# sampotter/butterfly

Hardware: AMD Instinct MI355X
Metric: butterfly matvecs/sec (2D Helmholtz HODBF apply) (higher is better)
Workload: dtype c128

## Files before the change

### butterfly_amd/csrc/bfhip_device.hip

```cpp

#include <hip/hip_runtime.h>
#include <type_traits>
#include <vector>
#include <stdint.h>
#include <stdio.h>
#include <stdlib.h>

#include "bfhip_internal.h"
#include "bfhip_stage_c128.h"
#include "../../include/bfhip_abi.h"
#include "../../include/bfhip_synth.h"

#define BF_WAVES_PER_WG 4
#define BF_WAVE_LDS_BYTES (BF_XCAP * 16)

static int hipFail(hipError_t e, char const *what) {
  if (e == hipSuccess) return 0;
  int code = (e == hipErrorOutOfMemory) ? BFABI_ERROR_MEMORY_ERROR : BFABI_ERROR_RUNTIME_ERROR;
  return bfhipFail(code, "%s: %s", what, hipGetErrorString(e));
}

struct __attribute__((aligned(8))) bfC64 { float re, im; };
struct bfC64Acc { double re, im; };
__device__ __forceinline__ bfC64Acc &operator+=(bfC64Acc &a, bfC64Acc b) { a.re += b.re; a.im += b.im; return a; }
// ... 519 lines not shown
            bool dual = pi + pstep < wn;
            BfDevPiece pc2 = pc;
            if (dual) {
              pc2 = bfPieceWinGet(win, pi + pstep);
              dual = (pc2.flags & (BF_PIECE_ROWMAJOR | BF_PIECE_IDENTITY)) == BF_PIECE_ROWMAJOR;
            }
            U a[ITERS], a2[ITERS];
            S xv[ITERS][NC], xv2[ITERS][NC];
#pragma unroll
            for (int i = 0; i < ITERS; ++i) {
              uint32_t const srow = rlRm + (uint32_t)i * RL_RM, sc = srow < n ? srow : n - 1;
              a[i] = bfLoadStreamV(src + (uint64_t)sc * rowUnits);
#pragma unroll
              for (int k = 0; k < NC; ++k) {
                S const xr = xin[(uint64_t)sc * nrhs * NC + k];
                xv[i][k] = srow < n ? xr : (S)0;
              }
            }
            if (dual) {
              S const *xin2 = ((pc2.flags & BF_PIECE_IN_X) ? (S const *)p.x : (S const *)p.temp) + ((uint64_t)pc2.inOff * nrhs + q) * NC;
              uint32_t const n2 = pc2.ncols;
              U const *src2 = arena + pc2.dataOff / EPL + cgc;
              uint32_t const rowUnits2 = pc2.ld / EPL;
#pragma unroll
              for (int i = 0; i < ITERS; ++i) {
                uint32_t const srow = rlRm + (uint32_t)i * RL_RM, sc = srow < n2 ? srow : n2 - 1;
                a2[i] = bfLoadStreamV(src2 + (uint64_t)sc * rowUnits2);
#pragma unroll
                for (int k = 0; k < NC; ++k) {
                  S const xr = xin2[(uint64_t)sc * nrhs * NC + k];
                  xv2[i][k] = srow < n2 ? xr : (S)0;
                }
              }
            }
#pragma unroll
            for (int i = 0; i < ITERS; ++i)
#pragma unroll
              for (int e = 0; e < EPL; ++e) bfMacN<NC>(racc[e], &a[i].v[e * NC], xv[i]);
            if (dual) {
#pragma unroll
              for (int i = 0; i < ITERS; ++i)
#pragma unroll
                for (int e = 0; e < EPL; ++e) bfMacN<NC>(racc[e], &a2[i].v[e * NC], xv2[i]);
              pi += pstep;
            }
            continue;
          }
        }
        uint32_t const stride = pc.ld / EPL;
        uint32_t const n = pc.ncols;
        uint32_t const units = (n + EPL - 1) / EPL;
        U const *src = arena + pc.dataOff / EPL;
        for (uint32_t rb = 0; rb < units; rb += R) {
          uint32_t const ru = rb + r < units ? rb + r : units - 1;
          U a[NQ];
#pragma unroll
          for (int cq = 0; cq < NQ; ++cq) if ((uint32_t)cq < nq) a[cq] = (R >= 16 || BF_T_WIDE_NT) ? bfLoadStreamV(src + jcol[cq] * stride + ru) : src[jcol[cq] * stride + ru];
          S xv[UNIT];
#pragma unroll
          for (int e = 0; e < EPL; ++e) {
            uint32_t const row = (rb + r) * EPL + e;
            uint32_t const rowc = row < n ? row : n - 1;
#pragma unroll
            for (int k = 0; k < NC; ++k) {
              S const v = xin[(uint64_t)rowc * nrhs * NC + k];
              xv[e * NC + k] = row < n ? v : (S)0;
            }
          }
#pragma unroll
          for (int cq = 0; cq < NQ; ++cq) {
            if ((uint32_t)cq >= nq) continue;
#pragma unroll
            for (int e = 0; e < EPL; ++e) bfMacN<NC>(acc[cq], &a[cq].v[e * NC], &xv[e * NC]);
          }
        }
      }
    }
#pragma unroll
    for (int m = 1; m < R; m <<= 1)
#pragma unroll
      for (int cq = 0; cq < NQ; ++cq)
#pragma unroll
        for (int k = 0; k < NC; ++k) acc[cq][k] += __shfl_xor(acc[cq][k], m, R);
    if constexpr (EPL > 1) {
      if (anyRowMajor) {
#pragma unroll
        for (int e = 0; e < EPL; ++e)
#pragma unroll
          for (int k = 0; k < NC; ++k)
#pragma unroll
            for (int m = CG_RM; m < 64; m <<= 1) racc[e][k] += __shfl_xor(racc[e][k], m, 64);
#pragma unroll
        for (int cq = 0; cq < NQ; ++cq) {
          uint32_t const col = c4 + C * cq < mr ? c4 + C * cq : 0;
#pragma unroll
          for (int e = 0; e < EPL; ++e)
#pragma unroll
            for (int k = 0; k < NC; ++k) {
              A const t = __shfl(racc[e][k], (int)(col / EPL), 64);
              if ((int)(col % EPL) == e) acc[cq][k] += t;
            }
        }
      }
    }
    if (COOP && coop) {
      if (r == 0) {
#pragma unroll
        for (int cq = 0; cq < NQ; ++cq)
#pragma unroll
          for (int k = 0; k < NC; ++k) coopBuf[wave][c4 + C * cq][k] = acc[cq][k];
      }
      __syncthreads();
      if (wave == 0 && r == 0) {
#pragma unroll
        for (int cq = 0; cq < NQ; ++cq)
#pragma unroll
          for (int k = 0; k < NC; ++k) {
            A t = coopBuf[0][c4 + C * cq][k];
#pragma unroll
            for (int w = 1; w < BF_WAVES_PER_WG; ++w) t += coopBuf[w][c4 + C * cq][k];
            acc[cq][k] = t;
          }
      }
      __syncthreads();
      if (wave != 0) continue;
    }
    if (r == 0) {
#pragma unroll
      for (int cq = 0; cq < NQ; ++cq)
        if (c4 + C * cq < mr)
#pragma unroll
          for (int k = 0; k < NC; ++k) out[(((uint64_t)it.outOff + c4 + C * cq) * nrhs + q) * NC + k] = (S)acc[cq][k];
    }
  }
}

template <int DT, int R, int NQ, bool COOP, bool ONE>
__global__ __launch_bounds__(BF_WAVES_PER_WG * 64) void bfStageKernelT(StageParams p) {
  using A = typename Traits<DT>::A;
  constexpr int NC = Traits<DT>::CPLX ? 2 : 1;
  __shared__ A coopBuf[COOP ? BF_WAVES_PER_WG : 1][COOP ? NQ * (64 / R) : 1][NC];
  bfStageBodyT<DT, R, NQ, COOP, ONE>(p, blockIdx.x, coopBuf);
}

template <int DT, bool ONE>
__global__ __launch_bounds__(BF_WAVES_PER_WG * 64) void bfStageKernelTBoth(StageParams pn, StageParams pw, uint32_t gridNarrow) {
  using A = typename Traits<DT>::A;
  constexpr int NC = Traits<DT>::CPLX ? 2 : 1;
  __shared__ A coopBuf[BF_WAVES_PER_WG][64][NC];
  if (blockIdx.x < gridNarrow) bfStageBodyT<DT, 16, 4, true, ONE>(pn, blockIdx.x, coopBuf);
  else bfStageBodyT<DT, BF_T_WIDE_R, BF_T_WIDE_R, true, ONE>(pw, blockIdx.x - gridNarrow, coopBuf);
}

struct ReduceBatch {
  uint32_t count, nrhs;
  void const *temp;
  struct Entry {
    uint32_t const *rowInterval, *ivBegin;
    int64_t const *srcBias;
    uint64_t numRows;
    void *dest;
    uint32_t blockBegin, pad;
  } e[BF_REDUCE_BATCH];
};

template <typename T, int NC, bool LONG = false>
__global__ __launch_bounds__(256) void bfReduceKernel(ReduceBatch const B) {
  using TA = typename std::conditional<NC == 2 && sizeof(T) == 4, double, T>::type;
  uint32_t k = 0;
  while (k + 1 < B.count && B.e[k + 1].blockBegin <= blockIdx.x) ++k;
  ReduceBatch::Entry const &E = B.e[k];
  uint32_t const nrhs = B.nrhs;
  uint64_t idx = (uint64_t)(blockIdx.x - E.blockBegin) * 256 + threadIdx.x;
  uint64_t total = E.numRows * nrhs;
  if (idx >= total) return;
  uint64_t row = idx / nrhs;
  uint32_t q = (uint32_t)(idx - row * nrhs);
  uint32_t iv = E.rowInterval[row];
  if (iv == 0xffffffffu) return;
  uint32_t b = E.ivBegin[iv], e = E.ivBegin[iv + 1];
  T const *temp = (T const *)B.temp;
  T *dest = (T *)E.dest;
  TA acc[NC];
#pragma unroll
  for (int c = 0; c < NC; ++c) acc[c] = 0;
  uint32_t s = b;
  if (LONG) {
    for (; s + 32 <= e; s += 32) {
      T v[32][NC];
#pragma unroll
      for (int k = 0; k < 32; ++k) {
        T const *src = temp + ((uint64_t)(E.srcBias[s + k] + (int64_t)row) * nrhs + q) * NC;
#pragma unroll
        for (int c = 0; c < NC; ++c) v[k][c] = src[c];
      }
#pragma unroll
      for (int k = 0; k < 32; ++k)
#pragma unroll
        for (int c = 0; c < NC; ++c) acc[c] += v[k][c];
    }
  }
#pragma unroll 8
  for (; s < e; ++s) {
    T const *src = temp + ((uint64_t)(E.srcBias[s] + (int64_t)row) * nrhs + q) * NC;
#pragma unroll
    for (int c = 0; c < NC; ++c) acc[c] += src[c];
  }
#pragma unroll
  for (int c = 0; c < NC; ++c) dest[idx * NC + c] = (T)acc[c];
}

template <typename S>
__global__ __launch_bounds__(256) void bfScalePermuteKernel(S *dst, S const *src, S const *scale, int power, uint64_t const *perm, uint64_t n) {
  uint64_t const i = (uint64_t)blockIdx.x * 256 + threadIdx.x;
  if (i >= n) return;
  S v = src[i];
  if (scale) { S const g = scale[i]; v *= power == 2 ? g * g : g; }
  uint64_t const j = perm ? perm[i] : i;
  if (j < n) dst[j] = v;
}

template <int DT>
__global__ __launch_bounds__(256) void bfSynthKernel(void *arenaV, BfSynthPiece const *pieces, uint64_t seed) {
  using S = typename Traits<DT>::S;
  constexpr bool CPLX = Traits<DT>::CPLX;
  BfSynthPiece const pc = pieces[blockIdx.x];
  uint64_t total = pc.rowMajor ? (uint64_t)pc.mr * pc.ldr : (uint64_t)pc.mrPad * pc.ncols;
  S *dst = (S *)arenaV + pc.dataOff * (CPLX ? 2 : 1);
  for (uint64_t e = threadIdx.x; e < total; e += 256) {
    uint32_t col, r;
    if (pc.rowMajor) { r = (uint32_t)(e / pc.ldr); col = (uint32_t)(e - (uint64_t)r * pc.ldr); }
    else { col = (uint32_t)(e / pc.mrPad); r = (uint32_t)(e - (uint64_t)col * pc.mrPad); }
    S re = 0, im = 0;
    if (r < pc.mr && col < pc.ncols) {
      uint64_t idx = pc.vbase + (uint64_t)(pc.row0 + r) * pc.strideR + (uint64_t)(pc.col0 + col) * pc.strideC;
      re = (S)(bfhip_synth_value(seed, idx, 0) * pc.scale);
      if (CPLX) im = (S)(bfhip_synth_value(seed, idx, 1) * pc.scale);
    }
    if (CPLX) { dst[2 * e] = re; dst[2 * e + 1] = im; }
    else dst[e] = re;
  }
}


#define BF_REAL_CASES(DT, NAME) \
  case BFHIP_KERNEL_REAL_##NAME: hipLaunchKernelGGL(bfStageKernelReal<DT>, dim3(grid), dim3(BF_WAVES_PER_WG * 64), 0, s, p); break; \
  case BFHIP_KERNEL_SMALL_##NAME: hipLaunchKernelGGL(bfStageKernelSmall<DT>, dim3(grid), dim3(BF_WAVES_PER_WG * 64), 0, s, p); break; \
  case BFHIP_KERNEL_REALBOTH_##NAME: hipLaunchKernelGGL(bfStageKernelRealBoth<DT>, dim3(grid + grid2), dim3(BF_WAVES_PER_WG * 64), 0, s, p, p2, grid); break;
#define BF_T_CASES(DT, NAME) \
  case BFHIP_KERNEL_T_##NAME##_NARROW_N: hipLaunchKernelGGL((bfStageKernelT<DT, 16, 4, false, false>), dim3(grid), dim3(BF_WAVES_PER_WG * 64), 0, s, p); break; \
  case BFHIP_KERNEL_T_##NAME##_NARROW_ONE: hipLaunchKernelGGL((bfStageKernelT<DT, 16, 4, false, true>), dim3(grid), dim3(BF_WAVES_PER_WG * 64), 0, s, p); break; \
  case BFHIP_KERNEL_T_##NAME##_NARROW_COOP_N: hipLaunchKernelGGL((bfStageKernelT<DT, 16, 4, true, false>), dim3(grid), dim3(BF_WAVES_PER_WG * 64), 0, s, p); break; \
  case BFHIP_KERNEL_T_##NAME##_NARROW_COOP_ONE: hipLaunchKernelGGL((bfStageKernelT<DT, 16, 4, true, true>), dim3(grid), dim3(BF_WAVES_PER_WG * 64), 0, s, p); break; \
  case BFHIP_KERNEL_T_##NAME##_WIDE_N: hipLaunchKernelGGL((bfStageKernelT<DT, BF_T_WIDE_R, BF_T_WIDE_R, false, false>), dim3(grid), dim3(BF_WAVES_PER_WG * 64), 0, s, p); break; \
  case BFHIP_KERNEL_T_##NAME##_WIDE_ONE: hipLaunchKernelGGL((bfStageKernelT<DT, BF_T_WIDE_R, BF_T_WIDE_R, false, true>), dim3(grid), dim3(BF_WAVES_PER_WG * 64), 0, s, p); break; \
  case BFHIP_KERNEL_T_##NAME##_WIDE_COOP_N: hipLaunchKernelGGL((bfStageKernelT<DT, BF_T_WIDE_R, BF_T_WIDE_R, true, false>), dim3(grid), dim3(BF_WAVES_PER_WG * 64), 0, s, p); break; \
  case BFHIP_KERNEL_T_##NAME##_WIDE_COOP_ONE: hipLaunchKernelGGL((bfStageKernelT<DT, BF_T_WIDE_R, BF_T_WIDE_R, true, true>), dim3(grid), dim3(BF_WAVES_PER_WG * 64), 0, s, p); break;
#define BF_TBOTH_CASES(DT, NAME) \
  case BFHIP_KERNEL_TBOTH_##NAME##_N: hipLaunchKernelGGL((bfStageKernelTBoth<DT, false>), dim3(grid + grid2), dim3(BF_WAVES_PER_WG * 64), 0, s, p, p2, grid); break; \
  case BFHIP_KERNEL_TBOTH_##NAME##_ONE: hipLaunchKernelGGL((bfStageKernelTBoth<DT, true>), dim3(grid + grid2), dim3(BF_WAVES_PER_WG * 64), 0, s, p, p2, grid); break;
static int bfLaunchWaveStage(BfKernelLaunch const &L, BfLaunchArgs const *a, StageParams p, hipStream_t s) {
  bool const small = L.kernel >= BFHIP_KERNEL_SMALL_F64 && L.kernel <= BFHIP_KERNEL_SMALL_C64;
  uint32_t const perWg = small ? 4 * BF_WAVES_PER_WG : BF_WAVES_PER_WG;
  p.items = (BfDevItem const *)a->items + L.first[0];
  p.numItems = (uint32_t)L.count[0];
  p.coopItems = (uint32_t)L.coop[0];
  uint32_t const grid = (uint32_t)(L.coop[0] + (L.count[0] - L.coop[0] + perWg - 1) / perWg);
  StageParams p2 = p;
  uint32_t grid2 = 0;
  if (L.numRanges == 2) {
    bool const tboth = L.kernel >= BFHIP_KERNEL_TBOTH_F64_N && L.kernel <= BFHIP_KERNEL_TBOTH_C64_ONE;
    uint32_t const perWg2 = tboth ? BF_WAVES_PER_WG : 4 * BF_WAVES_PER_WG;
    p2.items = (BfDevItem const *)a->items + L.first[1];
    p2.numItems = (uint32_t)L.count[1];
    p2.coopItems = (uint32_t)L.coop[1];
    grid2 = (uint32_t)(L.coop[1] + (L.count[1] - L.coop[1] + perWg2 - 1) / perWg2);
  }
  switch (L.kernel) {
    BF_REAL_CASES(BFHIP_F64, F64) BF_REAL_CASES(BFHIP_F32, F32) BF_REAL_CASES(BFHIP_C64, C64)
    BF_T_CASES(BFHIP_C128, C128) BF_T_CASES(BFHIP_F64, F64) BF_T_CASES(BFHIP_F32, F32) BF_T_CASES(BFHIP_C64, C64)
    BF_TBOTH_CASES(BFHIP_F64, F64) BF_TBOTH_CASES(BFHIP_F32, F32) BF_TBOTH_CASES(BFHIP_C64, C64)
    default: return bfhipFail(BFABI_ERROR_RUNTIME_ERROR, "internal: kernel id %u is not a wavefront-per-item stage kernel", L.kernel);
  }
  return 0;
}
#undef BF_REAL_CASES
#undef BF_T_CASES
#undef BF_TBOTH_CASES

extern "C" {

int bfdevSetDevice(int device) {
  if (device < 0) return 0;
  return hipFail(hipSetDevice(device), "hipSetDevice");
}
int bfdevGetDevice(int *device) { return hipFail(hipGetDevice(device), "hipGetDevice"); }
int bfdevMalloc(void **p, size_t bytes) {
  *p = NULL;
  if (!bytes) bytes = 16;
  return hipFail(hipMalloc(p, bytes), "hipMalloc");
}
void bfdevFree(void *p) { if (p) (void)hipFree(p); }
int bfdevMemcpyH2D(void *dst, void const *src, size_t bytes) { return bytes ? hipFail(hipMemcpy(dst, src, bytes, hipMemcpyHostToDevice), "hipMemcpy H2D") : 0; }
int bfdevMemcpyD2H(void *dst, void const *src, size_t bytes) { return bytes ? hipFail(hipMemcpy(dst, src, bytes, hipMemcpyDeviceToHost), "hipMemcpy D2H") : 0; }
int bfdevMemset(void *dst, int value, size_t bytes) { return bytes ? hipFail(hipMemset(dst, value, bytes), "hipMemset") : 0; }
int bfdevSync(void *stream) { return hipFail(hipStreamSynchronize((hipStream_t)stream), "hipStreamSynchronize"); }
int bfdevPointerKind(void const *p) {
  hipPointerAttribute_t a;
  hipError_t const e = hipPointerGetAttributes(&a, p);
  if (e != hipSuccess) { (void)hipGetLastError(); return 0; }
  if (a.type == hipMemoryTypeDevice) {
    int cur = -1;
    (void)hipGetDevice(&cur);
    return a.device == cur ? 1 : 3;
  }
  if (a.type == hipMemoryTypeHost) return 2;
  return 0;
}
int bfdevHostRegister(void *p, size_t bytes) { return hipFail(hipHostRegister(p, bytes, hipHostRegisterDefault), "hipHostRegister"); }
int bfdevHostUnregister(void *p) { return hipFail(hipHostUnregister(p), "hipHostUnregister"); }
int bfdevMemcpyAnyAsync(void *dst, void const *src, size_t bytes, void *stream) { return bytes ? hipFail(hipMemcpyAsync(dst, src, bytes, hipMemcpyDefault, (hipStream_t)stream), "hipMemcpyAsync") : 0; }
int bfdevHostAllocPinned(void **p, size_t bytes) { return hipFail(hipHostMalloc(p, bytes, hipHostMallocDefault), "hipHostMalloc"); }
void bfdevHostFreePinned(void *p) { if (p) (void)hipHostFree(p); }

int bfdevSynthFill(void *arena, uint32_t dtype, BfSynthPiece const *hostPieces, uint64_t count, uint64_t seed) {
  if (!count) return 0;
  BfSynthPiece *d = NULL;
  int rc = hipFail(hipMalloc((void **)&d, count * sizeof(BfSynthPiece)), "hipMalloc(synth pieces)");
  if (rc) return rc;
  rc = hipFail(hipMemcpy(d, hostPieces, count * sizeof(BfSynthPiece), hipMemcpyHostToDevice), "hipMemcpy(synth pieces)");
  if (!rc) {
    uint64_t done = 0;
    while (done < count && !rc) {
      uint32_t n = (uint32_t)((count - done) > (1u << 23) ? (1u << 23) : (count - done));
      if (dtype == BFHIP_C128) hipLaunchKernelGGL(bfSynthKernel<BFHIP_C128>, dim3(n), dim3(256), 0, 0, arena, d + done, seed);
      else if (dtype == BFHIP_F64) hipLaunchKernelGGL(bfSynthKernel<BFHIP_F64>, dim3(n), dim3(256), 0, 0, arena, d + done, seed);
      else if (dtype == BFHIP_C64) hipLaunchKernelGGL(bfSynthKernel<BFHIP_C64>, dim3(n), dim3(256), 0, 0, arena, d + done, seed);
      else hipLaunchKernelGGL(bfSynthKernel<BFHIP_F32>, dim3(n), dim3(256), 0, 0, arena, d + done, seed);
      rc = hipFail(hipGetLastError(), "synth fill launch");
      done += n;
    }
    if (!rc) rc = hipFail(hipDeviceSynchronize(), "synth fill");
  }
  (void)hipFree(d);
  return rc;
}

int bfdevLaunchStage(BfLaunchArgs const *a, void *stream) {
  if (!a->numItems) return 0;
  if (a->numItems >= (1ull << 32) / 256) return bfhipFail(BFABI_ERROR_RUNTIME_ERROR, "stage of %llu items exceeds the 32-bit global size of a launch", (unsigned long long)a->numItems);
  StageParams p;
  p.arena = a->arena;
  p.items = (BfDevItem const *)a->items;
  p.pieces = (BfDevPiece const *)a->pieces;
  p.numItems = (uint32_t)a->numItems;
  p.nrhs = a->nrhs;
  p.coopItems = 0;
  p.x = a->x;
  p.y = a->y;
  p.temp = a->temp;
  p.zero = a->zero;
  hipStream_t s = (hipStream_t)stream;
  if (!bfDtypeKnown(a->dtype)) return bfhipFail(BFABI_ERROR_TYPE_ERROR, "unknown dtype %u", a->dtype);
  BfKernelLaunch L[2];
  uint32_t const nl = bfSelectStageKernels(a, L);
  for (uint32_t i = 0; i < nl; ++i) {
    if (L[i].kernel == BFHIP_KERNEL_C128) {
      uint32_t const grid = (uint32_t)((a->numItems + BF_C128_WG_WAVES - 1) / BF_C128_WG_WAVES);
#ifdef BFHIP_EXPERIMENTAL
      { int handled = 0; int const rcx = bfdevLaunchStageExperimental(a, &p, grid, stream, &handled); if (handled) return rcx; }
#endif
      hipLaunchKernelGGL(bfStageKernelC128, dim3(grid), dim3(BF_C128_WG_WAVES * 64), 0, s, p);
    }
    else if (L[i].kernel >= BFHIP_KERNEL_EXT_BASE) {
      uint32_t const wg = L[i].kernel >= BFHIP_KERNEL_T_EXT_BASE ? BF_TM_WG_WAVES : 1;
      dim3 const g((uint32_t)((a->numItems + wg - 1) / wg)), b(64 * wg);
#define BF_BLK_CASES(ID, KERNEL, W2, W4, ...) \
        case ID##_MFMA1: hipLaunchKernelGGL((KERNEL<__VA_ARGS__ __VA_OPT__(,) 1, 4>), g, b, 0, s, p); break; \
        case ID##_MFMA2: hipLaunchKernelGGL((KERNEL<__VA_ARGS__ __VA_OPT__(,) 2, W2>), g, b, 0, s, p); break; \
        case ID##_MFMA4: hipLaunchKernelGGL((KERNEL<__VA_ARGS__ __VA_OPT__(,) 4, W4>), g, b, 0, s, p); break;
      switch (L[i].kernel) {
        BF_BLK_CASES(BFHIP_KERNEL_C64, bfStageKernelC64Mfma, 3, 2)
        BF_BLK_CASES(BFHIP_KERNEL_F64, bfStageKernelRealMfma, 4, 4, BFHIP_F64) BF_BLK_CASES(BFHIP_KERNEL_F32, bfStageKernelRealMfma, 4, 4, BFHIP_F32)
        BF_BLK_CASES(BFHIP_KERNEL_T_C128, bfStageKernelTMfma, 4, 2, BFHIP_C128) BF_BLK_CASES(BFHIP_KERNEL_T_F64, bfStageKernelTMfma, 4, 4, BFHIP_F64)
        BF_BLK_CASES(BFHIP_KERNEL_T_F32, bfStageKernelTMfma, 4, 4, BFHIP_F32) BF_BLK_CASES(BFHIP_KERNEL_T_C64, bfStageKernelTMfma, 4, 2, BFHIP_C64)
        default: return bfhipFail(BFABI_ERROR_RUNTIME_ERROR, "internal: kernel id %u is not a stage kernel", L[i].kernel);
      }
#undef BF_BLK_CASES
    }
    else if (L[i].kernel <= BFHIP_KERNEL_C128_MFMA4_EXACT) {
      dim3 const g((uint32_t)((a->numItems + BF_MF_WG_WAVES - 1) / BF_MF_WG_WAVES)), b(64 * BF_MF_WG_WAVES);
      switch (L[i].kernel) {
        case BFHIP_KERNEL_C128_MFMA1_EXACT: hipLaunchKernelGGL(bfStageKernelC128Mfma1Exact, g, b, 0, s, p); break;
        case BFHIP_KERNEL_C128_MFMA2_EXACT: hipLaunchKernelGGL(bfStageKernelC128Mfma2Exact, g, b, 0, s, p); break;
        case BFHIP_KERNEL_C128_MFMA4_EXACT: hipLaunchKernelGGL(bfStageKernelC128MfmaExact, g, b, 0, s, p); break;
        case BFHIP_KERNEL_C128_MFMA1: hipLaunchKernelGGL(bfStageKernelC128Mfma1, g, b, 0, s, p); break;
        case BFHIP_KERNEL_C128_MFMA2: hipLaunchKernelGGL(bfStageKernelC128Mfma2, g, b, 0, s, p); break;
        default: hipLaunchKernelGGL(bfStageKernelC128Mfma, g, b, 0, s, p); break;
      }
    }
    else {
      int const rc = bfLaunchWaveStage(L[i], a, p, s);
      if (rc) return rc;
    }
  }
  return hipFail(hipGetLastError(), a->transposed ? "transposed stage launch" : "stage launch");
}


int bfdevMemsetAsync(void *dst, int value, size_t bytes, void *stream) { return bytes ? hipFail(hipMemsetAsync(dst, value, bytes, (hipStream_t)stream), "hipMemsetAsync") : 0; }

int bfdevScalePermute(void *dst, void const *src, void const *scale, int power, uint64_t const *perm, uint64_t n, uint32_t dtype, void *stream) {
  if (!n) return 0;
  uint32_t const grid = (uint32_t)((n + 255) / 256);
  if (dtype == BFHIP_F64) hipLaunchKernelGGL(bfScalePermuteKernel<double>, dim3(grid), dim3(256), 0, (hipStream_t)stream, (double *)dst, (double const *)src, (double const *)scale, power, perm, n);
  else if (dtype == BFHIP_F32) hipLaunchKernelGGL(bfScalePermuteKernel<float>, dim3(grid), dim3(256), 0, (hipStream_t)stream, (float *)dst, (float const *)src, (float const *)scale, power, perm, n);
  else return bfhipFail(BFABI_ERROR_TYPE_ERROR, "scale/permute: real element types only");
  return hipFail(hipGetLastError(), "scale/permute launch");
}

int bfdevLaunchReduce(BfReduceArgs const *a, uint32_t count, void *stream) {
  hipStream_t s = (hipStream_t)stream;
  for (uint32_t base = 0; base < count; base += BF_REDUCE_BATCH) {
    ReduceBatch B;
    B.count = count - base < BF_REDUCE_BATCH ? count - base : BF_REDUCE_BATCH;
    B.nrhs = a[base].nrhs;
    B.temp = a[base].temp;
    uint32_t blocks = 0;
    for (uint32_t k = 0; k < B.count; ++k) {
      BfReduceArgs const *r = &a[base + k];
      B.e[k].rowInterval = (uint32_t const *)r->rowInterval; B.e[k].ivBegin = (uint32_t const *)r->ivBegin;
      B.e[k].srcBias = (int64_t const *)r->srcBias; B.e[k].numRows = r->numRows; B.e[k].dest = r->dest;
      B.e[k].blockBegin = blocks; B.e[k].pad = 0;
      blocks += (uint32_t)((r->numRows * r->nrhs + 255) / 256);
    }
    if (!blocks) continue;
    uint32_t const dtype = a[base].dtype;
    bool longLists = false;
    for (uint32_t k = 0; k < B.count; ++k) longLists = longLists || a[base + k].longLists;
    switch (bfSelectReduceKernel(dtype, longLists)) {
// ... 31 lines not shown
```

### butterfly_amd/csrc/bfhip_file.c

```c
#include "bfhip_operator.h"
#include "../../include/bfhip_abi.h"

#include <stdio.h>
#include <stdlib.h>
#include <string.h>

#define BFHIP_FILE_MAGIC "BFHIPOP1"

typedef struct FileHeader {
  char magic[8];
  uint32_t version, dtype, srcDtype, elemSize, epl, xcap, hasTplan, reserved;
  uint64_t numRows, numCols, arenaElems, leafElems, numLeaves, leafBytesAlgorithmic;
} FileHeader;

typedef struct FilePlanHeader { uint64_t numStages, tempElems, numRows, numCols; uint32_t maxItemRows, transposed; } FilePlanHeader;
typedef struct FileStageHeader { uint64_t numItems, numPieces, leafElems, vecIn, vecOut, numReduce; uint32_t maxRows, reserved; } FileStageHeader;
typedef struct FileReduceHeader { uint64_t destOff, numRows, numIntervals, numSrc; uint32_t destSpace, reserved; } FileReduceHeader;

static int writeAll(FILE *fp, void const *p, size_t n) { return n == 0 || fwrite(p, 1, n, fp) == n ? 0 : bfhipFail(BFABI_ERROR_FILE_ERROR, "short write"); }
static int readAll(FILE *fp, void *p, size_t n) { return n == 0 || fread(p, 1, n, fp) == n ? 0 : bfhipFail(BFABI_ERROR_FILE_ERROR, "short read / truncated file"); }

static int writeDeviceArray(FILE *fp, void const *d, size_t bytes) {
  if (!bytes) return 0;
  size_t const chunk = (size_t)64 << 20;
  void *h = malloc(bytes < chunk ? bytes : chunk);
  if (!h) return bfhipFail(BFABI_ERROR_MEMORY_ERROR, "host OOM");
  int rc = 0;
  for (size_t off = 0; off < bytes && !rc; off += chunk) {
    size_t n = bytes - off < chunk ? bytes - off : chunk;
    rc = bfdevMemcpyD2H(h, (char const *)d + off, n);
    if (!rc) rc = writeAll(fp, h, n);
  }
  free(h);
  return rc;
}
static int readDeviceArray(FILE *fp, void **d, size_t bytes, uint64_t *meta) {
  int rc = bfdevMalloc(d, bytes + BF_ARENA_SLACK);
  if (rc || !bytes) return rc;
  if (meta) *meta += bytes;
  size_t const chunk = (size_t)64 << 20;
  void *h = malloc(bytes < chunk ? bytes : chunk);
  if (!h) return bfhipFail(BFABI_ERROR_MEMORY_ERROR, "host OOM");
  for (size_t off = 0; off < bytes && !rc; off += chunk) {
    size_t n = bytes - off < chunk ? bytes - off : chunk;
    rc = readAll(fp, h, n);
    if (!rc) rc = bfdevMemcpyH2D((char *)*d + off, h, n);
  }
  free(h);
  return rc;
}

static int savePlan(FILE *fp, BfPlan const *pl) {
  FilePlanHeader ph = {pl->numStages, pl->tempElems, pl->numRows, pl->numCols, pl->maxItemRows, (uint32_t)pl->transposed};
  int rc = writeAll(fp, &ph, sizeof ph);
  for (uint64_t s = 0; s < pl->numStages && !rc; ++s) {
    BfStage const *st = &pl->stages[s];
    FileStageHeader sh = {st->numItems, st->numPieces, st->leafElems, st->vecIn, st->vecOut, st->numReduce, st->maxRows, 0};
    rc = writeAll(fp, &sh, sizeof sh);
    if (!rc) rc = writeDeviceArray(fp, st->dItems, st->numItems * sizeof(BfDevItem));
    if (!rc) rc = writeDeviceArray(fp, st->dPieces, st->numPieces * sizeof(BfDevPiece));
    for (uint64_t r = 0; r < st->numReduce && !rc; ++r) {
      BfReduce const *rd = &st->reduce[r];
      FileReduceHeader rh = {rd->destOff, rd->numRows, rd->numIntervals, rd->numSrc, rd->destSpace, 0};
      rc = writeAll(fp, &rh, sizeof rh);
      if (!rc) rc = writeDeviceArray(fp, rd->dRowInterval, rd->numRows * 4);
      if (!rc) rc = writeDeviceArray(fp, rd->dIvBegin, (rd->numIntervals + 1) * 4);
      if (!rc) rc = writeDeviceArray(fp, rd->dSrcBias, rd->numSrc * 8);
    }
  }
  return rc;
}

static int readMetaArray(FILE *fp, void **d, void **h, size_t bytes, uint64_t *meta) {
  *h = NULL;
  int rc = bfdevMalloc(d, bytes);
  if (rc || !bytes) return rc;
  if (meta) *meta += bytes;
  *h = malloc(bytes);
  if (!*h) return bfhipFail(BFABI_ERROR_MEMORY_ERROR, "host OOM");
  if ((rc = readAll(fp, *h, bytes))) return rc;
  return bfdevMemcpyH2D(*d, *h, bytes);
}

static int fitsIn(uint64_t off, uint64_t ext, uint64_t len) { return off <= len && ext <= len - off; }
static uint64_t mulAddSat(uint64_t a, uint64_t b, uint64_t c) {
  uint64_t r;
  if (__builtin_mul_overflow(a, b, &r) || __builtin_add_overflow(r, c, &r)) return UINT64_MAX;
  return r;
}

static int validateStage(BfPlan const *pl, uint64_t arenaElems, BfStage const *st, BfDevItem const *items, BfDevPiece const *pieces) {
  uint64_t const inX = pl->numCols, outY = pl->numRows, temp = pl->tempElems;
  for (uint64_t i = 0; i < st->numItems; ++i) {
    BfDevItem const *it = &items[i];
    uint32_t const mr = it->mrFlags & 0xffffu;
    uint64_t const outLen = (it->mrFlags & BF_ITEM_OUT_Y) ? outY : temp;
    if (!mr || mr > pl->maxItemRows || mr > st->maxRows || (it->mrFlags & ~(0xffffu | BF_ITEM_OUT_Y | BF_ITEM_ROWMAJOR | BF_ITEM_MERGED | BF_ITEM_SMALL | BF_ITEM_TNARROW)) ||
        ((it->mrFlags & BF_ITEM_TNARROW) != 0) != (i < st->numNarrow) || ((it->mrFlags & BF_ITEM_TNARROW) && (!pl->transposed || mr > 16)) ||
        ((it->mrFlags & BF_ITEM_SMALL) != 0) != (i >= st->firstSmall) ||
        ((it->mrFlags & BF_ITEM_ROWMAJOR) && (pl->transposed || bfDtypeC128Layout(pl->dtype) || mr > 2 * pl->epl)) ||
        (pl->transposed && mr > 64) ||
        !fitsIn(it->outOff, mr, outLen) || !fitsIn(it->pieceBegin, it->numPieces, st->numPieces))
      return bfhipFail(BFABI_ERROR_FILE_ERROR, "corrupt operator file: item %llu out of bounds", (unsigned long long)i);
    uint32_t const mrPad = (mr + pl->epl - 1) / pl->epl * pl->epl;
    if (it->mrFlags & (BF_ITEM_MERGED | BF_ITEM_SMALL)) {
      int const sm = (it->mrFlags & BF_ITEM_SMALL) != 0;
      uint64_t next = 0, dense = 0;
      int const smRm = sm && (it->mrFlags & BF_ITEM_ROWMAJOR);
      int badm = pl->transposed || bfDtypeC128Layout(pl->dtype) || (!sm && (it->mrFlags & BF_ITEM_ROWMAJOR)) || it->numPieces > (sm ? BF_SMALL_PIECES : 64u) ||
                 (sm && (mr > 2 * pl->epl || !(it->mrFlags & BF_ITEM_ROWMAJOR)));
      for (uint32_t k = 0; k < it->numPieces && !badm; ++k) {
        BfDevPiece const *pc = &pieces[it->pieceBegin + k];
        if (pc->flags & BF_PIECE_IDENTITY) continue;
        if (!smRm && dense && pc->dataOff != next) badm = 1;
        next = mulAddSat(mrPad, pc->ncols, pc->dataOff); dense += pc->ncols;
      }
      if (badm || (!dense && !sm) || dense > (sm ? BF_SMALL_COLS : BF_MERGE_COLS))
        return bfhipFail(BFABI_ERROR_FILE_ERROR, "corrupt operator file: merged item %llu is not one block", (unsigned long long)i);
    }
    for (uint32_t k = 0; k < it->numPieces; ++k) {
      BfDevPiece const *pc = &pieces[it->pieceBegin + k];
      uint64_t const inLen = (pc->flags & BF_PIECE_IN_X) ? inX : temp;
      int bad = (pc->flags & ~(BF_PIECE_IN_X | BF_PIECE_IDENTITY | BF_PIECE_ROWMAJOR)) != 0;
      int const rm = (pc->flags & BF_PIECE_ROWMAJOR) != 0;
      if (!(pc->flags & BF_PIECE_IDENTITY) && !pl->transposed && rm != ((it->mrFlags & BF_ITEM_ROWMAJOR) != 0)) bad = 1;
      if (pc->flags & BF_PIECE_IDENTITY) bad |= !fitsIn(pc->inOff, mr, inLen);
      else if (pl->transposed && rm)
        bad |= !pc->ld || pc->ld % pl->epl || pc->dataOff % pl->epl || bfDtypeC128Layout(pl->dtype) || !pc->ncols ||
               !fitsIn(pc->dataOff, mulAddSat(pc->ncols - 1, pc->ld, (mr + pl->epl - 1) / pl->epl * pl->epl), arenaElems) ||
               !fitsIn(pc->inOff, pc->ncols, inLen);
      else if (rm)
        bad |= !pc->ncols || pc->ld % pl->epl || pc->ld < pc->ncols || pc->dataOff % pl->epl ||
               !fitsIn(pc->dataOff, mulAddSat(mr, pc->ld, 0), arenaElems) || !fitsIn(pc->inOff, pc->ncols, inLen);
      else if (pl->transposed)
        bad |= !pc->ld || pc->ld % pl->epl || pc->ncols > pc->ld || pc->dataOff % pl->epl ||
               !fitsIn(pc->dataOff, mulAddSat(mr - 1, pc->ld, (pc->ncols + pl->epl - 1) / pl->epl * pl->epl), arenaElems) ||
               !fitsIn(pc->inOff, pc->ncols, inLen);
      else
        bad |= !pc->ncols || pc->ncols > pl->xcap || pc->dataOff % pl->epl ||
               !fitsIn(pc->dataOff, mulAddSat(mrPad, pc->ncols, 0), arenaElems) || !fitsIn(pc->inOff, pc->ncols, inLen);
      if (bad) return bfhipFail(BFABI_ERROR_FILE_ERROR, "corrupt operator file: piece %u of item %llu out of bounds", k, (unsigned long long)i);
    }
  }
  return 0;
}

static int validateReduce(BfPlan const *pl, BfReduce const *rd, uint32_t const *rowInterval, uint32_t const *ivBegin, int64_t const *srcBias) {
  uint64_t const destLen = rd->destSpace == BF_SPACE_Y ? pl->numRows : pl->tempElems;
  if ((rd->destSpace != BF_SPACE_Y && rd->destSpace != BF_SPACE_TEMP) || !fitsIn(rd->destOff, rd->numRows, destLen) || rd->numIntervals > rd->numRows + 1)
    return bfhipFail(BFABI_ERROR_FILE_ERROR, "corrupt operator file: reduce destination out of bounds");
  if (ivBegin[0] != 0 || ivBegin[rd->numIntervals] > rd->numSrc) return bfhipFail(BFABI_ERROR_FILE_ERROR, "corrupt operator file: reduce interval table");
  for (uint64_t i = 0; i < rd->numIntervals; ++i)
    if (ivBegin[i + 1] < ivBegin[i]) return bfhipFail(BFABI_ERROR_FILE_ERROR, "corrupt operator file: reduce interval table not monotone");
  for (uint64_t r = 0; r < rd->numRows; ++r) {
    uint32_t const iv = rowInterval[r];
    if (iv == BF_REDUCE_SKIP) continue;
    if (iv >= rd->numIntervals) return bfhipFail(BFABI_ERROR_FILE_ERROR, "corrupt operator file: reduce row %llu", (unsigned long long)r);
    for (uint32_t k = ivBegin[iv]; k < ivBegin[iv + 1]; ++k) {
      int64_t src;
      if (__builtin_add_overflow(srcBias[k], (int64_t)r, &src) || src < 0 || (uint64_t)src >= pl->tempElems) return bfhipFail(BFABI_ERROR_FILE_ERROR, "corrupt operator file: reduce source out of bounds");
    }
  }
  return 0;
}

static int loadPlan(FILE *fp, BfhipOperator *op, BfPlan *pl, FileHeader const *fh, uint64_t arenaElems) {
  FilePlanHeader ph;
  int rc = readAll(fp, &ph, sizeof ph);
  if (rc) return rc;
  if (ph.numStages > (1u << 20) || ph.tempElems >= 0xffffffffu) return bfhipFail(BFABI_ERROR_FILE_ERROR, "corrupt plan header");
  pl->dtype = fh->dtype; pl->elemSize = fh->elemSize; pl->epl = fh->epl; pl->xcap = fh->xcap;
  pl->maxItemRows = ph.maxItemRows; pl->transposed = (int)ph.transposed;
  pl->numRows = ph.numRows; pl->numCols = ph.numCols; pl->numStages = ph.numStages; pl->tempElems = ph.tempElems;
  pl->arenaElems = pl->transposed ? 0 : arenaElems;
  pl->leafElems = fh->leafElems; pl->numLeaves = fh->numLeaves;
  if (pl->epl != 16 / pl->elemSize || pl->xcap != 256 || pl->maxItemRows > 64 * pl->epl || (pl->transposed && pl->maxItemRows > 128))
    return bfhipFail(BFABI_ERROR_FILE_ERROR, "corrupt plan header (lane granule / piece width / item height)");
  pl->stages = calloc(ph.numStages ? ph.numStages : 1, sizeof(BfStage));
  if (!pl->stages) return bfhipFail(BFABI_ERROR_MEMORY_ERROR, "host OOM");
  for (uint64_t s = 0; s < pl->numStages && !rc; ++s) {
    BfStage *st = &pl->stages[s];
    FileStageHeader sh;
    if ((rc = readAll(fp, &sh, sizeof sh))) break;
    if (sh.numItems > 0xffffffffu || sh.numPieces > 0xffffffffu || sh.numReduce > (1u << 20)) { rc = bfhipFail(BFABI_ERROR_FILE_ERROR, "corrupt stage header"); break; }
    st->numItems = sh.numItems; st->numPieces = sh.numPieces; st->leafElems = sh.leafElems; st->vecIn = sh.vecIn; st->vecOut = sh.vecOut;
    st->maxRows = sh.maxRows;
    void *hItems = NULL, *hPieces = NULL;
    rc = readMetaArray(fp, &st->dItems, &hItems, st->numItems * sizeof(BfDevItem), &op->metaBytes);
    if (!rc) rc = readMetaArray(fp, &st->dPieces, &hPieces, st->numPieces * sizeof(BfDevPiece), &op->metaBytes);
    if (!rc) {
      st->firstSmall = st->numItems;
      while (st->firstSmall && (((BfDevItem const *)hItems)[st->firstSmall - 1].mrFlags & BF_ITEM_SMALL)) --st->firstSmall;
      st->numNarrow = 0;
      while (st->numNarrow < st->numItems && (((BfDevItem const *)hItems)[st->numNarrow].mrFlags & BF_ITEM_TNARROW)) ++st->numNarrow;
      rc = validateStage(pl, arenaElems, st, hItems, hPieces);
      if (!rc && pl->transposed) {
        st->maxRowsRest = 0;
        for (uint64_t i = st->numNarrow; i < st->numItems; ++i) {
          uint32_t const mr = ((BfDevItem const *)hItems)[i].mrFlags & 0xffffu;
          if (mr > st->maxRowsRest) st->maxRowsRest = mr;
        }
        st->numCoopNarrow = bfPlanCountCoop(hItems, hPieces, st->numNarrow, pl->elemSize);
        st->numCoop = bfPlanCountCoop((BfDevItem const *)hItems + st->numNarrow, hPieces, st->numItems - st->numNarrow, pl->elemSize);
      }
    }
    free(hItems); free(hPieces);
    if (!rc && sh.numReduce) {
      st->reduce = calloc(sh.numReduce, sizeof(BfReduce));
      if (!st->reduce) rc = bfhipFail(BFABI_ERROR_MEMORY_ERROR, "host OOM");
    }
    for (uint64_t r = 0; r < sh.numReduce && !rc; ++r) {
      BfReduce *rd = &st->reduce[r];
      FileReduceHeader rh;
      if ((rc = readAll(fp, &rh, sizeof rh))) break;
      st->numReduce = r + 1;
      rd->destOff = rh.destOff; rd->numRows = rh.numRows; rd->numIntervals = rh.numIntervals; rd->numSrc = rh.numSrc; rd->destSpace = rh.destSpace;
      if (rd->numRows >= 0xffffffffu || rd->numIntervals >= 0xffffffffu || rd->numSrc >= 0xffffffffu) { rc = bfhipFail(BFABI_ERROR_FILE_ERROR, "corrupt reduce header"); break; }
      void *hRow = NULL, *hIv = NULL, *hBias = NULL;
      rc = readMetaArray(fp, &rd->dRowInterval, &hRow, rd->numRows * 4, &op->metaBytes);
      if (!rc) rc = readMetaArray(fp, &rd->dIvBegin, &hIv, (rd->numIntervals + 1) * 4, &op->metaBytes);
      if (!rc) rc = readMetaArray(fp, &rd->dSrcBias, &hBias, rd->numSrc * 8, &op->metaBytes);
      if (!rc) rc = validateReduce(pl, rd, hRow, hIv, hBias);
      if (!rc) {
        uint32_t const *iv = hIv;
        rd->maxSrc = 0;
        for (uint64_t i = 0; i < rd->numIntervals; ++i) if (iv[i + 1] - iv[i] > rd->maxSrc) rd->maxSrc = iv[i + 1] - iv[i];
      }
      free(hRow); free(hIv); free(hBias);
    }
  }
  return rc;
}

int bfhipSave(BfhipOperator *op, char const *path) {
  if (!op || !path) return bfhipFail(BFABI_ERROR_INVALID_ARGUMENTS, "NULL argument");
  if (op->flags & BFHIP_FLAG_PLAN_ONLY) return bfhipFail(BFABI_ERROR_RUNTIME_ERROR, "a plan-only operator has no device data to save");
  int prev = -1;
  bfdevGetDevice(&prev);
  int rc = bfdevSetDevice(op->device);
  if (rc) return rc;
  if ((rc = bfdevSync(NULL))) return rc;
  FILE *fp = fopen(path, "wb");
  if (!fp) return bfhipFail(BFABI_ERROR_FILE_ERROR, "cannot open %s for writing", path);
  FileHeader fh;
  memset(&fh, 0, sizeof fh);
  memcpy(fh.magic, BFHIP_FILE_MAGIC, 8);
  fh.version = 1; fh.dtype = op->plan.dtype; fh.srcDtype = op->srcDtype; fh.elemSize = op->plan.elemSize; fh.epl = op->plan.epl;
  fh.xcap = op->plan.xcap; fh.hasTplan = (uint32_t)op->hasTplan;
  fh.reserved = op->dArenaT ? 1u : 0u;
  fh.numRows = op->plan.numRows; fh.numCols = op->plan.numCols; fh.arenaElems = op->plan.arenaElems;
  fh.leafElems = op->plan.leafElems; fh.numLeaves = op->plan.numLeaves; fh.leafBytesAlgorithmic = op->leafBytesAlgorithmic;
  rc = writeAll(fp, &fh, sizeof fh);
  uint64_t const arenaElemsT = op->dArenaT ? op->tplan.arenaElems : 0;
  if (!rc && op->dArenaT) rc = writeAll(fp, &arenaElemsT, sizeof arenaElemsT);
  if (!rc) rc = savePlan(fp, &op->plan);
  if (!rc && op->hasTplan) rc = savePlan(fp, &op->tplan);
  if (!rc) rc = writeDeviceArray(fp, op->dArena, (size_t)op->plan.arenaElems * op->plan.elemSize);
  if (!rc && op->dArenaT) rc = writeDeviceArray(fp, op->dArenaT, (size_t)arenaElemsT * op->plan.elemSize);
  if (fclose(fp) != 0 && !rc) rc = bfhipFail(BFABI_ERROR_FILE_ERROR, "error closing %s", path);
  if (prev >= 0 && prev != op->device) bfdevSetDevice(prev);
  return rc;
}

int bfhipLoad(char const *path, BfhipOptions const *opts, BfhipOperator **out) {
  if (!path || !out) return bfhipFail(BFABI_ERROR_INVALID_ARGUMENTS, "NULL argument");
  *out = NULL;
  BfhipOptions o;
  memset(&o, 0, sizeof o);
  o.device = -1;
  if (opts) {
    if (opts->structSize < BFHIP_OPTIONS_SIZE_V1) return bfhipFail(BFABI_ERROR_INVALID_ARGUMENTS, "BfhipOptions.structSize too small");
    memcpy(&o, opts, opts->structSize < sizeof o ? opts->structSize : sizeof o);
  }
  if (o.flags & BFHIP_FLAG_PLAN_ONLY) return bfhipFail(BFABI_ERROR_INVALID_ARGUMENTS, "cannot load as plan-only");
  FILE *fp = fopen(path, "rb");
  if (!fp) return bfhipFail(BFABI_ERROR_FILE_ERROR, "cannot open %s", path);
  FileHeader fh;
  int rc = readAll(fp, &fh, sizeof fh);
  if (!rc && (memcmp(fh.magic, BFHIP_FILE_MAGIC, 8) != 0 || fh.version != 1 || fh.dtype > BFHIP_C64 ||
              fh.elemSize != bfDtypeElemSize(fh.dtype) || (fh.dtype == BFHIP_C64 && fh.srcDtype != BFHIP_C128)))
    rc = bfhipFail(BFABI_ERROR_FILE_ERROR, "%s is not a bfhip operator file (bad magic / version / dtype)", path);
  if (rc) { fclose(fp); return rc; }
  BfhipOperator *op = calloc(1, sizeof *op);
  if (!op) { fclose(fp); return bfhipFail(BFABI_ERROR_MEMORY_ERROR, "host OOM"); }
  int prevDev = -1;
  bfdevGetDevice(&prevDev);
  op->flags = o.flags & ~(uint32_t)(BFHIP_FLAG_ADJOINT | BFHIP_FLAG_ADJOINT_PACKED);
  op->srcDtype = fh.srcDtype;
// ... 26 lines not shown
```

Before: 96.16.

## Add lean c128 transposed stage kernel with two-tile software prefetch

Adds a specialised c128 transposed-stage kernel for single-RHS launches. It walks the pieces as a flat tile stream, issuing loads for the next tile before consuming the current one (depth 2). It uses 32-bit byte offsets and branch-free select logic in place of the generic path. A file validator check rejects leading dimensions of 2^22 or more so the 32-bit offsets cannot overflow. The aim is to cut load latency stalls and register/control overhead, at the cost of extra register pressure from double-buffered tiles.

```diff
diff --git a/butterfly_amd/csrc/bfhip_device.hip b/butterfly_amd/csrc/bfhip_device.hip
--- a/butterfly_amd/csrc/bfhip_device.hip
+++ b/butterfly_amd/csrc/bfhip_device.hip
@@ -695,6 +695,11 @@
   else bfStageBodyT<DT, BF_T_WIDE_R, BF_T_WIDE_R, true, ONE>(pw, blockIdx.x - gridNarrow, coopBuf);
 }
 
+#ifndef BF_T_C128_LEAN
+#define BF_T_C128_LEAN 2
+#endif
+#include "bfhip_stage_t_c128.h"
+
 struct ReduceBatch {
   uint32_t count, nrhs;
   void const *temp;
@@ -799,6 +804,20 @@
   case BFHIP_KERNEL_T_##NAME##_WIDE_ONE: hipLaunchKernelGGL((bfStageKernelT<DT, BF_T_WIDE_R, BF_T_WIDE_R, false, true>), dim3(grid), dim3(BF_WAVES_PER_WG * 64), 0, s, p); break; \
   case BFHIP_KERNEL_T_##NAME##_WIDE_COOP_N: hipLaunchKernelGGL((bfStageKernelT<DT, BF_T_WIDE_R, BF_T_WIDE_R, true, false>), dim3(grid), dim3(BF_WAVES_PER_WG * 64), 0, s, p); break; \
   case BFHIP_KERNEL_T_##NAME##_WIDE_COOP_ONE: hipLaunchKernelGGL((bfStageKernelT<DT, BF_T_WIDE_R, BF_T_WIDE_R, true, true>), dim3(grid), dim3(BF_WAVES_PER_WG * 64), 0, s, p); break;
+#if BF_T_C128_LEAN
+#define BF_T_C128_ONE(R, NQ, COOP) bfStageKernelTLean<R, NQ, COOP, BF_T_C128_LEAN>
+#else
+#define BF_T_C128_ONE(R, NQ, COOP) bfStageKernelT<BFHIP_C128, R, NQ, COOP, true>
+#endif
+#define BF_T_C128_CASES \
+  case BFHIP_KERNEL_T_C128_NARROW_N: hipLaunchKernelGGL((bfStageKernelT<BFHIP_C128, 16, 4, false, false>), dim3(grid), dim3(BF_WAVES_PER_WG * 64), 0, s, p); break; \
+  case BFHIP_KERNEL_T_C128_NARROW_ONE: hipLaunchKernelGGL((BF_T_C128_ONE(16, 4, false)), dim3(grid), dim3(BF_WAVES_PER_WG * 64), 0, s, p); break; \
+  case BFHIP_KERNEL_T_C128_NARROW_COOP_N: hipLaunchKernelGGL((bfStageKernelT<BFHIP_C128, 16, 4, true, false>), dim3(grid), dim3(BF_WAVES_PER_WG * 64), 0, s, p); break; \
+  case BFHIP_KERNEL_T_C128_NARROW_COOP_ONE: hipLaunchKernelGGL((BF_T_C128_ONE(16, 4, true)), dim3(grid), dim3(BF_WAVES_PER_WG * 64), 0, s, p); break; \
+  case BFHIP_KERNEL_T_C128_WIDE_N: hipLaunchKernelGGL((bfStageKernelT<BFHIP_C128, BF_T_WIDE_R, BF_T_WIDE_R, false, false>), dim3(grid), dim3(BF_WAVES_PER_WG * 64), 0, s, p); break; \
+  case BFHIP_KERNEL_T_C128_WIDE_ONE: hipLaunchKernelGGL((BF_T_C128_ONE(BF_T_WIDE_R, BF_T_WIDE_R, false)), dim3(grid), dim3(BF_WAVES_PER_WG * 64), 0, s, p); break; \
+  case BFHIP_KERNEL_T_C128_WIDE_COOP_N: hipLaunchKernelGGL((bfStageKernelT<BFHIP_C128, BF_T_WIDE_R, BF_T_WIDE_R, true, false>), dim3(grid), dim3(BF_WAVES_PER_WG * 64), 0, s, p); break; \
+  case BFHIP_KERNEL_T_C128_WIDE_COOP_ONE: hipLaunchKernelGGL((BF_T_C128_ONE(BF_T_WIDE_R, BF_T_WIDE_R, true)), dim3(grid), dim3(BF_WAVES_PER_WG * 64), 0, s, p); break;
 #define BF_TBOTH_CASES(DT, NAME) \
   case BFHIP_KERNEL_TBOTH_##NAME##_N: hipLaunchKernelGGL((bfStageKernelTBoth<DT, false>), dim3(grid + grid2), dim3(BF_WAVES_PER_WG * 64), 0, s, p, p2, grid); break; \
   case BFHIP_KERNEL_TBOTH_##NAME##_ONE: hipLaunchKernelGGL((bfStageKernelTBoth<DT, true>), dim3(grid + grid2), dim3(BF_WAVES_PER_WG * 64), 0, s, p, p2, grid); break;
@@ -821,7 +840,7 @@
   }
   switch (L.kernel) {
     BF_REAL_CASES(BFHIP_F64, F64) BF_REAL_CASES(BFHIP_F32, F32) BF_REAL_CASES(BFHIP_C64, C64)
-    BF_T_CASES(BFHIP_C128, C128) BF_T_CASES(BFHIP_F64, F64) BF_T_CASES(BFHIP_F32, F32) BF_T_CASES(BFHIP_C64, C64)
+    BF_T_C128_CASES BF_T_CASES(BFHIP_F64, F64) BF_T_CASES(BFHIP_F32, F32) BF_T_CASES(BFHIP_C64, C64)
     BF_TBOTH_CASES(BFHIP_F64, F64) BF_TBOTH_CASES(BFHIP_F32, F32) BF_TBOTH_CASES(BFHIP_C64, C64)
     default: return bfhipFail(BFABI_ERROR_RUNTIME_ERROR, "internal: kernel id %u is not a wavefront-per-item stage kernel", L.kernel);
   }
@@ -829,6 +848,7 @@
 }
 #undef BF_REAL_CASES
 #undef BF_T_CASES
+#undef BF_T_C128_CASES
 #undef BF_TBOTH_CASES
 
 extern "C" {
diff --git a/butterfly_amd/csrc/bfhip_file.c b/butterfly_amd/csrc/bfhip_file.c
--- a/butterfly_amd/csrc/bfhip_file.c
+++ b/butterfly_amd/csrc/bfhip_file.c
@@ -134,6 +134,7 @@
                !fitsIn(pc->dataOff, mulAddSat(mr, pc->ld, 0), arenaElems) || !fitsIn(pc->inOff, pc->ncols, inLen);
       else if (pl->transposed)
         bad |= !pc->ld || pc->ld % pl->epl || pc->ncols > pc->ld || pc->dataOff % pl->epl ||
+               (bfDtypeC128Layout(pl->dtype) && pc->ld >= (1u << 22)) ||
                !fitsIn(pc->dataOff, mulAddSat(mr - 1, pc->ld, (pc->ncols + pl->epl - 1) / pl->epl * pl->epl), arenaElems) ||
                !fitsIn(pc->inOff, pc->ncols, inLen);
       else
diff --git a/butterfly_amd/csrc/bfhip_stage_t_c128.h b/butterfly_amd/csrc/bfhip_stage_t_c128.h
--- /dev/null
+++ b/butterfly_amd/csrc/bfhip_stage_t_c128.h
@@ -0,0 +1,182 @@
+#ifndef BFHIP_STAGE_T_C128_H
+#define BFHIP_STAGE_T_C128_H
+
+struct BfTLeanDesc {
+  char const *base, *xin;
+  uint32_t stride, n, rb;
+  bool dense, add;
+};
+template <int NQ> struct BfTLeanTile {
+  bf_d2 a[NQ];
+  bf_d2 x;
+};
+
+template <bool NT> __device__ __forceinline__ bf_d2 bfTLeanLoad(char const *base, uint32_t byteOff) {
+  bf_d2 const *q = (bf_d2 const *)(base + byteOff);
+  if constexpr (NT && BF_STREAM_NT) return __builtin_nontemporal_load(q);
+  else return *q;
+}
+
+template <int R, int NQ, bool NT>
+__device__ __forceinline__ void bfTLeanIssue(BfTLeanTile<NQ> &t, BfTLeanDesc const &d, uint32_t const r, uint32_t const (&jcol)[NQ], uint32_t const nq) {
+  uint32_t const ru = d.rb + r < d.n ? d.rb + r : d.n - 1;
+#pragma unroll
+  for (int cq = 0; cq < NQ; ++cq) {
+    bool const used = (uint32_t)cq < nq;
+    t.a[cq] = bfTLeanLoad<NT>(used ? d.base : d.xin, used ? (jcol[cq] * d.stride + ru) << 4 : 0u);
+  }
+  t.x = bfTLeanLoad<false>(d.xin, ru << 4);
+}
+template <int R, int NQ>
+__device__ __forceinline__ void bfTLeanApply(BfTLeanTile<NQ> const &t, BfTLeanDesc const &d, double (&acc)[NQ][2], uint32_t const r) {
+  double xv[2] = {t.x.x, t.x.y};
+  uint32_t const lim = d.n - d.rb;
+  if (lim < (uint32_t)R) {
+    bool const live = r < lim;
+    xv[0] = live ? xv[0] : 0.0;
+    xv[1] = live ? xv[1] : 0.0;
+  }
+  bool const adds = d.add && r == 0;
+#pragma unroll
+  for (int cq = 0; cq < NQ; ++cq) {
+    double const a[2] = {t.a[cq].x, t.a[cq].y};
+    double f[2] = {acc[cq][0], acc[cq][1]};
+    bfMacN<2>(f, a, xv);
+    double const s0 = acc[cq][0] + a[0], s1 = acc[cq][1] + a[1];
+    double const k0 = adds ? s0 : acc[cq][0], k1 = adds ? s1 : acc[cq][1];
+    acc[cq][0] = d.dense ? f[0] : k0;
+    acc[cq][1] = d.dense ? f[1] : k1;
+  }
+}
+
+template <int R, int NQ, int DEPTH>
+__device__ __forceinline__ void bfTLeanChain(StageParams const &p, BfDevItem const &it, uint32_t const lane, uint32_t const wsel, uint32_t const pstep, double (&acc)[NQ][2]) {
+  constexpr int C = 64 / R;
+  constexpr bool NT = R >= 16 || BF_T_WIDE_NT;
+  static_assert(DEPTH == 1 || DEPTH == 2, "one or two tiles requested before the first is consumed");
+  using Tile = BfTLeanTile<NQ>;
+  uint32_t const mr = it.mrFlags & 0xffffu;
+  uint32_t const c4 = lane / R, r = lane % R;
+  uint32_t const nq = (mr + C - 1) / C;
+  uint32_t jcol[NQ];
+#pragma unroll
+  for (int cq = 0; cq < NQ; ++cq) jcol[cq] = c4 + C * cq < mr ? c4 + C * cq : mr - 1;
+
+  BfPieceWin win;
+  uint32_t pg = wsel;
+  BfTLeanDesc cur;
+  enum { BF_TL_END = 0, BF_TL_TILE = 1, BF_TL_WINDOW = 2 };
+  auto describe = [&]() {
+    BfDevPiece const pc = bfPieceWinGet(win, pg & 63u);
+    bool const ident = (pc.flags & BF_PIECE_IDENTITY) != 0;
+    bool const dense = !ident && pc.ncols;
+    char const *xin = (char const *)((pc.flags & BF_PIECE_IN_X) ? p.x : (void const *)p.temp) + (uint64_t)pc.inOff * 16;
+    cur.xin = dense || ident ? xin : (char const *)p.zero;
+    cur.base = dense ? (char const *)p.arena + pc.dataOff * 16 : cur.xin;
+    cur.stride = dense ? pc.ld : ident ? 1u : 0u;
+    cur.n = dense ? pc.ncols : 1u;
+    cur.rb = 0;
+    cur.dense = dense;
+    cur.add = ident;
+  };
+  auto step = [&]() -> int {
+    cur.rb += R;
+    if (cur.rb < cur.n) return BF_TL_TILE;
+    pg += pstep;
+    if (pg >= it.numPieces) return BF_TL_END;
+    if ((pg & 63u) < pstep) return BF_TL_WINDOW;
+    describe();
+    return BF_TL_TILE;
+  };
+
+  if (pg >= it.numPieces) return;
+  int st = BF_TL_WINDOW;
+  do {
+    if (st == BF_TL_WINDOW) {
+      uint32_t const wbase = pg & ~63u, wn = it.numPieces - wbase < 64u ? it.numPieces - wbase : 64u;
+      win = bfPieceWinLoad(p.pieces + it.pieceBegin + wbase, wn, (int)lane);
+      describe();
+    }
+    BfTLeanDesc const d0 = cur;
+    Tile t0;
+    bfTLeanIssue<R, NQ, NT>(t0, d0, r, jcol, nq);
+    if constexpr (DEPTH == 2) {
+      st = step();
+      bool const more = st == BF_TL_TILE;
+      BfTLeanDesc d1 = more ? cur : d0;
+      d1.dense = more && d1.dense;
+      d1.add = more && d1.add;
+      Tile t1;
+      bfTLeanIssue<R, NQ, NT>(t1, d1, r, jcol, nq);
+      bfTLeanApply<R, NQ>(t0, d0, acc, r);
+      bfTLeanApply<R, NQ>(t1, d1, acc, r);
+      if (more) st = step();
+    } else {
+      bfTLeanApply<R, NQ>(t0, d0, acc, r);
+      st = step();
+    }
+  } while (st != BF_TL_END);
+}
+
+template <int R, int NQ, bool COOP, int DEPTH, typename CoopBuf>
+__device__ __forceinline__ void bfStageBodyTLean(StageParams const &p, uint32_t const bid, CoopBuf &coopBuf) {
+  constexpr int C = 64 / R;
+  uint32_t const wave = __builtin_amdgcn_readfirstlane(threadIdx.x >> 6);
+  uint32_t const lane = threadIdx.x & 63;
+  bool const coop = COOP && bid < p.coopItems;
+  uint32_t const item = coop ? bid : p.coopItems + (bid - p.coopItems) * BF_WAVES_PER_WG + wave;
+  if (item >= p.numItems) return;
+  BfDevItem const it = p.items[item];
+  uint32_t const mr = it.mrFlags & 0xffffu;
+  uint32_t const c4 = lane / R, r = lane % R;
+  double acc[NQ][2];
+#pragma unroll
+  for (int cq = 0; cq < NQ; ++cq) acc[cq][0] = acc[cq][1] = 0;
+  uint32_t const wsel = coop ? wave : 0u, pstep = coop ? (uint32_t)BF_WAVES_PER_WG : 1u;
+  bfTLeanChain<R, NQ, DEPTH>(p, it, lane, wsel, pstep, acc);
+
+#pragma unroll
+  for (int m = 1; m < R; m <<= 1)
+#pragma unroll
+    for (int cq = 0; cq < NQ; ++cq)
+#pragma unroll
+      for (int k = 0; k < 2; ++k) acc[cq][k] += __shfl_xor(acc[cq][k], m, R);
+  if (COOP && coop) {
+    if (r == 0) {
+#pragma unroll
+      for (int cq = 0; cq < NQ; ++cq)
+#pragma unroll
+        for (int k = 0; k < 2; ++k) coopBuf[wave][c4 + C * cq][k] = acc[cq][k];
+    }
+    __syncthreads();
+    if (wave != 0) return;
+    if (r == 0) {
+#pragma unroll
+      for (int cq = 0; cq < NQ; ++cq)
+#pragma unroll
+        for (int k = 0; k < 2; ++k) {
+          double t = coopBuf[0][c4 + C * cq][k];
+#pragma unroll
+          for (int w = 1; w < BF_WAVES_PER_WG; ++w) t += coopBuf[w][c4 + C * cq][k];
+          acc[cq][k] = t;
+        }
+    }
+  }
+  if (r == 0) {
+    double *out = (it.mrFlags & BF_ITEM_OUT_Y) ? (double *)p.y : (double *)p.temp;
+#pragma unroll
+    for (int cq = 0; cq < NQ; ++cq)
+      if (c4 + C * cq < mr) {
+        bf_d2 const v = {acc[cq][0], acc[cq][1]};
+        *(bf_d2 *)(out + ((uint64_t)it.outOff + c4 + C * cq) * 2) = v;
+      }
+  }
+}
+
+template <int R, int NQ, bool COOP, int DEPTH>
+__global__ __launch_bounds__(BF_WAVES_PER_WG * 64) void bfStageKernelTLean(StageParams p) {
+  __shared__ double coopBuf[COOP ? BF_WAVES_PER_WG : 1][COOP ? NQ * (64 / R) : 1][2];
+  bfStageBodyTLean<R, NQ, COOP, DEPTH>(p, blockIdx.x, coopBuf);
+}
+
+#endif
```

Result: no change. 96.12 (-0.0%).
